# vision-agh/apse_uav

Measured on AMD Instinct MI355X. Metric: 4K UAV frames/sec (whole node), higher is better.
Workload: dtype f32

## Files before the change

### apse_uav_amd/_lib.py

```python
import ctypes as C
import os

import numpy as np

_HERE = os.path.dirname(os.path.abspath(__file__))
_TREE_LIB = os.path.join(_HERE, "libapse_hip.so")
LIB_PATH = os.environ.get("APSE_HIP_LIB") or _TREE_LIB
TOOL_ENTRIES = ("apse_winograd_pack_filter", "apse_winograd_conv2d", "apse_lane_stats")

APSE_OK = 0


class ApseError(RuntimeError):
    pass


class Config(C.Structure):
    _fields_ = [
        ("struct_size", C.c_int), ("device", C.c_int), ("max_batch", C.c_int),
        ("frame_h", C.c_int), ("frame_w", C.c_int), ("image_h", C.c_int), ("image_w", C.c_int),
        ("blocks", C.c_int * 4), ("num_classes", C.c_int),
        ("score_thresh", C.c_float), ("box_nms", C.c_float), ("rpn_nms", C.c_float), ("mask_thresh", C.c_float),
        ("rpn_pre_topk", C.c_int), ("rpn_post_topk", C.c_int), ("dets_per_image", C.c_int),
        ("pixel_mean", C.c_float * 3), ("assoc_roi", C.c_int), ("embed_dim", C.c_int), ("assoc_scale", C.c_float),
        ("compute_dtype", C.c_int), ("storage16", C.c_int),
    ]


class ConfigArch(Config):
    _fields_ = [("arch", C.c_int)]

# ... 44 lines not shown
    "apse_rpn_levels": ([vp, i, i, vp], i),
    "apse_box_head": ([vp, i, vp], i),
    "apse_set_detections": ([vp, vp, vp, vp, vp, i, vp], i),
    "apse_mask_tail": ([vp, i, vp], i),
    "apse_embed": ([vp, i, vp], i),
    "apse_forward": ([vp, i, vp], i),
    "apse_results_describe": ([vp, C.POINTER(ResultsLayout)], i),
    "apse_read_results": ([vp, vp, sz, vp], i),
    "apse_read_results_begin": ([vp, vp, sz, vp], i),
    "apse_read_results_end": ([vp, vp], i),
    "apse_lane_stats": ([vp, C.POINTER(C.c_longlong * 4)], i),
    "apse_copy_mask_window": ([vp, i, i, i, i, i, vp, vp], i),
    "apse_copy_mask_windows": ([vp, i, vp, vp, vp, vp, vp], i),
    "apse_host_copy": ([vp, vp, sz, i], i),
    "apse_feature_shape": ([vp, C.c_char_p, C.POINTER(C.c_int * 3)], i),
    "apse_export_feature": ([vp, C.c_char_p, vp, i, vp], i),
    "apse_debug_tensor": ([vp, C.c_char_p, vp, sz, C.POINTER(sz), vp], i),
    "apse_flops": ([vp, i, C.c_double, C.c_double], C.c_double),
    "apse_profile": ([vp, i], i),
    "apse_profile_read": ([vp, C.POINTER(C.c_double * 42), i], i),
    "apse_conv_packed_elems": ([C.POINTER(ConvDesc)], sz),
    "apse_conv_pack_weight": ([C.POINTER(ConvDesc), vp, i, vp, vp], i),
    "apse_conv2d": ([C.POINTER(ConvDesc), vp, vp, vp, vp, vp, vp, sz, vp], i),
    "apse_winograd_pack_filter": ([vp, i, i, vp], i),
    "apse_winograd_conv2d": ([C.POINTER(ConvDesc), vp, vp, vp, vp, vp], i),
    "apse_maxpool3x3s2": ([vp, vp, i, i, i, i, vp], i),
    "apse_maxpool3x3s2_typed": ([vp, vp, i, i, i, i, i, vp], i),
    "apse_roi_align": ([C.POINTER(vp), C.POINTER(i), C.POINTER(i), vp, i, i, i, vp, vp], i),
    "apse_roi_align_typed": ([C.POINTER(vp), C.POINTER(i), C.POINTER(i), vp, i, i, i, i, vp, vp], i),
    "apse_roi_pool": ([vp, i, i, vp, vp, i, i, f, vp, vp], i),
    "apse_roi_features": ([vp, i, vp, vp, i, i, vp, vp], i),
    "apse_nms_rank": ([vp, vp, vp, i, i, i, i, f, i, vp, vp, vp, vp, vp], i),
    "apse_mask_centroid_dense": ([vp, i, i, C.POINTER(C.c_int * 3), vp], i),
    "apse_mask_closest_dense": ([vp, i, i, f, f, C.POINTER(C.c_int * 2), vp], i),
    "apse_l2_normalize": ([vp, vp, i, i, vp], i),
    "apse_sqdist": ([vp, vp, i, i, i, vp, vp], i),
    "apse_undistort_gamma": ([vp, vp, i, i, i, C.POINTER(C.c_double), C.POINTER(C.c_double), i, vp, i, i, vp], i),
    "apse_lab_tables_host": ([vp, vp, C.c_size_t], C.c_size_t),
    "apse_replay_create": ([i, i, f, i], vp),
    "apse_replay_destroy": ([vp], None),
    "apse_replay_step": ([vp, i, i, vp, vp, vp, C.c_char_p, i, vp], i),
    "apse_replay_packed": ([vp, vp, C.c_longlong, i, i, i, vp, C.c_longlong], C.c_longlong),
    "apse_replay_max_id": ([vp], i),
    "apse_replay_next_id": ([vp], i),
    "apse_render_workspace_bytes": ([i, i, i], sz),
    "apse_render_instances": ([vp, vp, i, i, i, i, vp, i, vp, sz, vp, i, vp, sz, vp], i),
# ... 101 lines not shown
```

### apse_uav_amd/csrc/apse_common.h

```cpp
#pragma once
#include <hip/hip_runtime.h>
#include <stdint.h>

#define APSE_OK 0
#define APSE_E_INVALID (-1)
#define APSE_E_HIP (-2)
#define APSE_E_NOMEM (-3)
#define APSE_E_STATE (-4)
#define APSE_E_MISSING (-5)
#define APSE_MAX_FRAME_W 49152
#define APSE_MAX_FRAME_H 32768
#define APSE_MAX_CLASSES 80
#define APSE_LDS_BYTES 163840

int apse_fail_global(int code, const char* msg);

typedef __attribute__((ext_vector_type(16))) float f32x16;
typedef __attribute__((ext_vector_type(4))) float f32x4;

struct ConvParams {
    const float* x;
    const float* w;
    const uint16_t* w16;
    const float* bias;
// ... 14 lines not shown
    int out_mode;
    int y_ld, y_coff;
    int cdec;
    int splitk;
    int steps_total;
    const void* next_w;
    unsigned next_w_bytes;
    int prec;
    int x_st, res_st, y_st;
    int no_stream;
    const float* wu;
};

int apse_launch_conv(const ConvParams& p, int cfg, hipStream_t s, hipEvent_t ev0 = nullptr, hipEvent_t ev1 = nullptr);
int apse_conv_pick_cfg(int M, int Cout, int steps, int* splitk);
#define APSE_CFG_STREAM 9
#define APSE_CFG_BNECK 10
#define APSE_CFG_GLDS 11
#define APSE_CFG_STEMPOOL 12
#define APSE_CFG_SKINNY 13
#define APSE_NCFG 14
bool apse_conv1x1_stream_ok(const ConvParams& p);
int apse_launch_conv1x1_stream(const ConvParams& p, hipStream_t s, hipEvent_t ev0 = nullptr, hipEvent_t ev1 = nullptr);
bool apse_conv_glds16_ok(const ConvParams& p);
bool apse_conv_glds16_small(const ConvParams& p);
bool apse_conv_skinny_ok(const ConvParams& p);
int apse_launch_conv_skinny(const ConvParams& p, hipStream_t s, hipEvent_t ev0 = nullptr, hipEvent_t ev1 = nullptr);
int apse_launch_conv_glds16(const ConvParams& p, hipStream_t s, hipEvent_t ev0 = nullptr, hipEvent_t ev1 = nullptr);
int apse_conv_effective_cfg(const ConvParams& p, int cfg);
bool apse_conv_winograd_ok(const ConvParams& p, int max_items);
int apse_conv_winograd_blocks(const ConvParams& p);
int apse_launch_conv_winograd(const ConvParams& p, hipStream_t s, hipEvent_t ev0 = nullptr, hipEvent_t ev1 = nullptr);
typedef __bf16 bf16x8 __attribute__((ext_vector_type(8)));

#ifdef __HIPCC__
typedef _Float16 f16x4_t __attribute__((ext_vector_type(4)));
typedef __bf16 bf16x4_t __attribute__((ext_vector_type(4)));
__device__ __forceinline__ f32x4 apse_ld4(const void* base, size_t idx, int st) {
    if (st == 0) return *reinterpret_cast<const f32x4*>(reinterpret_cast<const float*>(base) + idx);
    f32x4 r;
    if (st == 1) {
        const uint2 raw = *reinterpret_cast<const uint2*>(reinterpret_cast<const uint16_t*>(base) + idx);
        r[0] = __uint_as_float(raw.x << 16); r[1] = __uint_as_float(raw.x & 0xffff0000u);
        r[2] = __uint_as_float(raw.y << 16); r[3] = __uint_as_float(raw.y & 0xffff0000u);
    } else {
        const f16x4_t h = *reinterpret_cast<const f16x4_t*>(reinterpret_cast<const uint16_t*>(base) + idx);
// ... 92 lines not shown
```

### apse_uav_amd/csrc/detector.hip

```cpp
#include "detector_ctx.h"

#include <math.h>
#include <string.h>

static std::string g_create_error;

int fail(apse_ctx* c, int code, const std::string& msg) {
    if (c) c->err = msg; else g_create_error = msg;
    return code;
}
int apse_fail_global(int code, const char* msg) { return fail(nullptr, code, msg); }

static int take_event_pair(apse_ctx* c, hipStream_t s) {
    if (!c->prof_on) return -1;
    if (c->ev_used == 0) {
        hipEventRecord(c->ev_pool[c->ev_base], s);
        hipEventRecord(c->ev_pool[c->ev_base + 1], s);
        c->ev_used = 2;
    }
    if (c->ev_used + 2 > APSE_EV_HALF) return -1;
    const int e0 = c->ev_base + c->ev_used;
    c->ev_used += 2;
    return e0;
}
// ... 73 lines not shown
    return APSE_OK;
}

static void count_lane_forward(apse_ctx* c, bool on) {
    if (!on || c->fwd_counted) return;
    ++c->lane_stats[0];
    c->fwd_counted = true;
}

static int run_plan(apse_ctx* c, std::vector<Step>& plan, int batch, hipStream_t s) {
    int* total_dev = reinterpret_cast<int*>(c->res + c->lay.total);
    int* propcnt_dev = reinterpret_cast<int*>(c->res + c->lay.prop_count);
    float* ws = (c->lane && s == c->lane) ? c->ws_lane : c->ws;
    for (size_t si = 0; si < plan.size(); ++si) {
        Step& st = plan[si];
        int rc = APSE_OK;
        if (&plan == &c->backbone && (int)si == c->fpn_step && c->lane && c->tail_live && !event_done(c->tail_ev)) {
            ++c->lane_stats[2];
            HIPCHK(c, hipStreamWaitEvent(s, c->tail_ev, 0));
        }
        if (st.kind == S_CONV) {
            ConvParams p = st.c.p;
            for (size_t sj = si + 1; sj < plan.size() && sj <= si + 2; ++sj)
                if (plan[sj].kind == S_CONV) {
                    const ConvParams& q = plan[sj].c.p;
                    const size_t elems = q.wu ? (size_t)16 * q.Cout * (1 << q.cin_log2) : (size_t)apse_roundup(q.Cout, 128) * q.KH * q.KWCp;
                    p.next_w = q.w16 ? (const void*)q.w16 : (q.wu ? (const void*)q.wu : (const void*)q.w);
                    const size_t bytes = elems * (q.w16 ? 2 : 4);
                    p.next_w_bytes = bytes > (64u << 20) ? (64u << 20) : (unsigned)bytes;
                    break;
                }
            p.B = st.c.fixed_items > 0 ? st.c.fixed_items : batch * st.c.b_mult;
            p.M = p.B * p.OH * p.OW;
            p.ws = ws;
            p.tile_cnt = nullptr;
            p.m_count = nullptr; p.m_per_item = p.OH * p.OW; p.m_hint = 0;
            int cfg = st.c.cfg;
            if (st.c.count_kind == 2) {
                p.m_count = total_dev;
                const int mh = (c->hint_total > 0 ? c->hint_total : 1) * p.m_per_item;
                p.m_hint = mh < p.M ? mh : p.M;
                if (p.prec != 0 && p.splitk == 1 && (cfg == 0 || cfg == 1 || cfg == 3)) {
                    int sk_dyn = 1;
                    const int cfg_dyn = apse_conv_pick_cfg(p.m_hint, p.Cout, p.steps_total, &sk_dyn);
                    if (sk_dyn == 1 && (cfg_dyn == 0 || cfg_dyn == 1 || cfg_dyn == 3)) cfg = cfg_dyn;
                }
            }
            else if (st.c.count_kind == 1 && batch == 1) p.m_count = propcnt_dev;
            const int e0 = take_event_pair(c, s);
            const hipEvent_t ev0 = e0 >= 0 ? c->ev_pool[e0] : nullptr, ev1 = e0 >= 0 ? c->ev_pool[e0 + 1] : nullptr;
            if (st.c.pool_y) {
                rc = apse_k_stem_pool16(p.x, p.w16, p.bias, st.c.pool_y, batch, p.H, p.W, p.prec, s, ev0, ev1);
                cfg = APSE_CFG_STEMPOOL;
            } else if (p.wu) {
                rc = apse_launch_conv_winograd(p, s, ev0, ev1);
            } else {
                rc = apse_launch_conv(p, cfg, s, ev0, ev1);
                cfg = apse_conv_effective_cfg(p, cfg);
            }
            if (e0 >= 0) c->pending.push_back({cfg, st.c.flops_per_item, st.c.count_kind, st.c.b_mult, batch, e0, e0 + 1});
        } else if (st.kind == S_BNECK) {
            const int e0 = take_event_pair(c, s);
            const ConvParams& q1 = st.c.p;
            rc = apse_k_bottleneck64_fused16(st.x, st.p3.res, st.y, q1.w16, q1.bias, st.p2.w16, st.p2.bias, st.p3.w16, st.p3.bias, batch,
                                             st.H, st.W, st.C, st.st, s, e0 >= 0 ? c->ev_pool[e0] : nullptr,
                                             e0 >= 0 ? c->ev_pool[e0 + 1] : nullptr);
            if (e0 >= 0) c->pending.push_back({APSE_CFG_BNECK, st.c.flops_per_item, 0, 1, batch, e0, e0 + 1});
        } else if (st.kind == S_MAXPOOL) {
            rc = apse_k_maxpool3x3s2(st.x, st.y, batch, st.H, st.W, st.C, st.st, s);
        } else {
            rc = apse_k_subsample2(st.x, st.y, batch, st.H, st.W, st.C, st.st, s);
        }
        if (rc != APSE_OK) return fail(c, rc, "launch failed at step " + st.c.name);
    }
    return APSE_OK;
}

int fill_camera(UndistortParams& p, int H, int W, const double* m, const double* dist, int ndist, int do_undistort, int do_gamma) {
    memset(&p, 0, sizeof p);
    if (!m || ndist > 14 || ndist < 0 || (ndist > 0 && !dist)) return APSE_E_INVALID;
    for (int i = 0; i < ndist && i < 12; ++i) p.k[i] = dist[i];
    if (ndist > 12 && (dist[12] != 0.0 || (ndist > 13 && dist[13] != 0.0))) return APSE_E_INVALID;
    const double a = m[0], b = m[1], c = m[2], dd = m[3], e = m[4], f = m[5], g = m[6], h = m[7], k = m[8];
    const double det = a * (e * k - f * h) - b * (dd * k - f * g) + c * (dd * h - e * g);
    if (det == 0.0) return APSE_E_INVALID;
    const double id = 1.0 / det;
    p.ir[0] = (e * k - f * h) * id; p.ir[1] = (c * h - b * k) * id; p.ir[2] = (b * f - c * e) * id;
    p.ir[3] = (f * g - dd * k) * id; p.ir[4] = (a * k - c * g) * id; p.ir[5] = (c * dd - a * f) * id;
    p.ir[6] = (dd * h - e * g) * id; p.ir[7] = (b * g - a * h) * id; p.ir[8] = (a * e - b * dd) * id;
    p.fx = m[0]; p.fy = m[4]; p.u0 = m[2]; p.v0 = m[5];
// ... 674 lines not shown
    else if (nm == "embedding_raw") { src = c->emb_raw; n = (size_t)B * g.dets_per_image * g.embed_dim * 4; }
    else {
        auto it = c->t.find(nm);
        if (it == c->t.end()) return fail(c, APSE_E_MISSING, "no tensor " + nm);
        const Tens& t = it->second;
        int items = B;
        if (nm == "box_pooled" || nm == "box_fc1" || nm == "box_fc2" || nm == "box_pred" || nm == "box_mean" || nm == "box_res5")
            items = B * g.rpn_post_topk;
        else if (nm.rfind("mask_", 0) == 0 || nm.rfind("assoc_", 0) == 0) items = B * g.dets_per_image;
        src = t.p; n = (size_t)items * t.H * t.W * t.C * (t.st ? 2 : 4);
    }
    if (bytes) *bytes = n;
    if (!dst) return APSE_OK;
    if (n > max_bytes) return fail(c, APSE_E_INVALID, "debug buffer too small for " + nm);
    int rc = lane_join(c, (hipStream_t)stream);
    if (rc) return rc;
    HIPCHK(c, hipMemcpyAsync(dst, src, n, hipMemcpyDeviceToDevice, (hipStream_t)stream));
    return lane_follow(c, (hipStream_t)stream);
}

double apse_flops(apse_ctx* c, int batch, double proposals, double detections) {
    if (!c || !c->finalized) return 0.0;
    double f = 0;
    for (auto& s : c->backbone) if (s.kind == S_CONV || s.kind == S_BNECK) f += s.c.flops_per_item * batch;
    for (auto& s : c->rpnhead) f += s.c.flops_per_item * batch;
    for (auto& s : c->c4_res5box) f += s.c.flops_per_item * proposals;
    for (auto& s : c->boxhead) f += s.c.flops_per_item * proposals;
    for (auto& s : c->maskhead) f += s.c.flops_per_item * detections;
    for (auto& s : c->embedfc) f += s.c.flops_per_item * detections;
    return f;
}

int apse_set_camera(apse_ctx* c, const double* m, const double* dist, int ndist, const uint8_t* lut_host, int do_undistort, int do_gamma) {
    if (!c) return APSE_E_INVALID;
    if (lane_drain(c)) return APSE_E_HIP;
    if (!do_undistort && !do_gamma) { c->cam_on = false; return APSE_OK; }
    if (do_gamma && !lut_host) return fail(c, APSE_E_INVALID, "gamma needs a 256-entry LUT");
    UndistortParams p;
    int rc = fill_camera(p, c->cfg.frame_h, c->cfg.frame_w, m, dist, ndist, do_undistort, do_gamma);
    if (rc) return fail(c, rc, "bad camera parameters (3x3 matrix, <= 14 distortion coefficients, tilt terms zero)");
    hipSetDevice(c->cfg.device);
    if (!c->cam_lut) {
        c->cam_lut = dalloc<LabTables>(c, 1);
        if (!c->cam_lut) return fail(c, APSE_E_NOMEM, "camera Lab tables alloc");
    }
    if (lut_host) {
        LabTables host;
// ... 26 lines not shown
```

### apse_uav_amd/csrc/detector_ctx.h

```cpp
#pragma once
#include "apse_kernels.h"
#include "../../include/apse_hip.h"
#include "preproc_pixel.h"

#include <map>
#include <string>
#include <vector>

#define APSE_NARROW_CLASSES 6
#define APSE_EV_HALF 1024

struct HostW { std::vector<float> v; std::vector<int64_t> shape; };
struct Tens { float* p = nullptr; int H = 0, W = 0, C = 0; int st = 0; };

struct ConvStep {
    ConvParams p;
    int b_mult = 1;
    int fixed_items = 0;
    int cfg = 0;
    double flops_per_item = 0;
    int count_kind = 0;
    void* pool_y = nullptr;
    std::string name;
};
enum StepKind { S_CONV, S_MAXPOOL, S_SUBSAMPLE, S_BNECK };
struct Step { StepKind kind; ConvStep c; const float* x; float* y; int H, W, C; int st = 0; ConvParams p2, p3; };

struct apse_ctx {
    apse_config cfg;
    std::string err;
    bool f32_winograd = true;
    std::map<std::string, HostW> hw;
    bool finalized = false;
    int PH = 0, PW = 0;
    std::vector<void*> allocs;
    std::map<std::string, Tens> t;
    std::vector<Step> backbone, rpnhead, boxhead, maskhead, embedfc;
    float* ws = nullptr; size_t ws_floats = 0; int* tile_cnt = nullptr;
    int *hb = nullptr, *hc = nullptr, *vb = nullptr, *vc = nullptr; int hk = 0, vk = 0; uint8_t* rs_tmp = nullptr;
    int rs_pitch = 0;
    int* hcT = nullptr;
    RpnLevels rl_host; RpnLevels* rl_dev = nullptr;
    std::vector<std::vector<TopkJob>> stages; std::vector<TopkJob*> stage_dev; int nslots = 0; uint64_t* lists = nullptr;
    int final_slot_host[5]; int* final_slot_dev = nullptr;
    float *dec_boxes = nullptr, *dec_scores = nullptr; int* dec_valid = nullptr; uint32_t* maxc = nullptr;
    int *keep_idx = nullptr, *keep_cnt = nullptr; void* nms_scratch = nullptr;
    float *props = nullptr, *prop_scores = nullptr; int *prop_entry = nullptr;
    FpnMaps fm;
// ... 68 lines not shown
```

### apse_uav_amd/csrc/ops.hip

```cpp
#include "detector_ctx.h"

#include <string.h>

#include <map>
#include <mutex>
#include <vector>

extern "C" {

size_t apse_conv_packed_elems(const apse_conv_desc* d) {
    const int cin_p = pow2_at_least(d->Cin);
    return (size_t)apse_roundup(d->Cout, 128) * d->KH * apse_roundup(d->KW * cin_p, 32);
}

int apse_conv_pack_weight(const apse_conv_desc* d, const float* w, int cin_real, const float* scale, float* packed) {
    if (!d || !w || !packed) return APSE_E_INVALID;
    const int cin_p = pow2_at_least(d->Cin);
    const int KWCp = apse_roundup(d->KW * cin_p, 32);
    memset(packed, 0, apse_conv_packed_elems(d) * sizeof(float));
    pack_oihw(w, d->Cout, cin_real, d->KH, d->KW, cin_p, scale, packed, KWCp);
    return APSE_OK;
}

int apse_conv2d(const apse_conv_desc* d, const float* x, const float* w, const float* bias, const float* res, float* y, float* ws,
                size_t ws_bytes, void* stream) {
    if (!d || !x || !w || !y) return APSE_E_INVALID;
    const int cin_p = pow2_at_least(d->Cin);
    if (cin_p != d->Cin) return APSE_E_INVALID;
    ConvParams p;
    memset(&p, 0, sizeof p);
    p.x = x; p.w = w; p.bias = bias; p.res = res; p.y = y; p.ws = ws;
    p.B = d->B; p.H = d->H; p.W = d->W; p.cin_log2 = apse_ilog2(cin_p);
    p.KH = d->KH; p.KW = d->KW; p.stride = d->stride; p.pad = d->pad;
    p.KWCp = apse_roundup(d->KW * cin_p, 32);
    p.OH = (d->H + 2 * d->pad - d->KH) / d->stride + 1;
    p.OW = (d->W + 2 * d->pad - d->KW) / d->stride + 1;
    p.Cout = d->Cout; p.relu = d->relu; p.res_mode = d->res_mode;
    p.M = p.B * p.OH * p.OW; p.m_per_item = p.OH * p.OW;
    p.y_ld = d->Cout; p.steps_total = p.KH * (p.KWCp / 32);
    p.prec = (d->prec == 1 || d->prec == 2) ? d->prec : 0;
    p.x_st = d->x_st; p.res_st = d->res_st; p.y_st = d->y_st;
    if (p.x_st < 0 || p.x_st > 2 || p.res_st < 0 || p.res_st > 2 || p.y_st < 0 || p.y_st > 2) return APSE_E_INVALID;
    if (p.prec && p.x_st && p.x_st != p.prec) return APSE_E_INVALID;
    if (p.x_st && cin_p < 8) return APSE_E_INVALID;
    int sk = 1;
    int cfg = apse_conv_pick_cfg(p.M, p.Cout, p.steps_total, &sk);
    if (d->cfg >= 0) { cfg = d->cfg; sk = 1; p.no_stream = (d->cfg != APSE_CFG_STREAM && d->cfg != APSE_CFG_GLDS && d->cfg != APSE_CFG_SKINNY); }
    if (d->splitk > 0) sk = d->splitk;
    if (sk > p.steps_total) sk = p.steps_total;
    p.splitk = sk;
    if (sk > 1 && (size_t)sk * p.M * p.Cout * sizeof(float) > ws_bytes) return APSE_E_INVALID;
    if (sk > 1 && d->fuse_reduce) {
        static int* cnt = nullptr;
        if (!cnt) { if (hipMalloc(reinterpret_cast<void**>(&cnt), 65536 * sizeof(int)) != hipSuccess) return APSE_E_NOMEM; hipMemset(cnt, 0, 65536 * sizeof(int)); }
        p.tile_cnt = cnt;
    }
    if (!p.prec) return apse_launch_conv(p, cfg, (hipStream_t)stream);
    const size_t ne = (size_t)apse_roundup(p.Cout, 128) * p.KH * p.KWCp;
    static uint16_t* d16 = nullptr;
    static size_t d16_cap = 0;
    if (ne > d16_cap) {
        hipDeviceSynchronize();
        if (d16) hipFree(d16);
        d16 = nullptr; d16_cap = 0;
        if (hipMalloc(reinterpret_cast<void**>(&d16), ne * 2) != hipSuccess) return APSE_E_NOMEM;
        d16_cap = ne;
    }
    int rc = apse_k_round16(w, d16, ne, p.prec, (hipStream_t)stream);
    if (rc) return rc;
    p.w16 = d16;
    return apse_launch_conv(p, cfg, (hipStream_t)stream);
}

int apse_winograd_pack_filter(const float* w, int Cout, int Cin, float* packed) {
    if (!w || !packed || Cout < 1 || Cin < 8 || pow2_at_least(Cin) != Cin) return APSE_E_INVALID;
    const std::vector<float> u = winograd_filters(w, Cout, Cin, Cin);
    memcpy(packed, u.data(), u.size() * sizeof(float));
    return APSE_OK;
}

int apse_winograd_conv2d(const apse_conv_desc* d, const float* x, const float* wu, const float* bias, float* y, void* stream) {
    if (!d || !x || !wu || !y || d->B < 1 || d->H < 1 || d->W < 1 || d->Cin < 8 || pow2_at_least(d->Cin) != d->Cin) return APSE_E_INVALID;
    ConvParams p;
    memset(&p, 0, sizeof p);
    p.x = x; p.wu = wu; p.bias = bias; p.y = y;
    p.B = d->B; p.H = d->H; p.W = d->W; p.cin_log2 = apse_ilog2(d->Cin);
    p.KH = d->KH; p.KW = d->KW; p.stride = d->stride; p.pad = d->pad;
    p.OH = d->H; p.OW = d->W; p.Cout = d->Cout; p.relu = d->relu;
    p.M = p.B * p.OH * p.OW; p.m_per_item = p.OH * p.OW;
    p.y_ld = d->Cout; p.splitk = 1;
    p.res_mode = d->res_mode; p.prec = d->prec; p.x_st = d->x_st; p.y_st = d->y_st;
    return apse_launch_conv_winograd(p, (hipStream_t)stream);
}

// ... 181 lines not shown
```

### apse_uav_amd/csrc/plan.hip

```cpp
#include "detector_ctx.h"

#include <math.h>
#include <stdio.h>
#include <string.h>

#define APSE_WINO_MIN_BLOCKS 128
#define APSE_EXPECTED_DETS 8

void pack_oihw(const float* w, int Cout, int Cin, int KH, int KW, int cin_p, const float* scale, float* out, int KWCp) {
    for (int o = 0; o < Cout; ++o) {
        const float sc = scale ? scale[o] : 1.0f;
        for (int r = 0; r < KH; ++r)
            for (int s = 0; s < KW; ++s)
                for (int ci = 0; ci < Cin; ++ci)
                    out[((size_t)o * KH + r) * KWCp + s * cin_p + ci] = w[(((size_t)o * Cin + ci) * KH + r) * KW + s] * sc;
    }
}

static const HostW* getw(apse_ctx* c, const std::string& n) {
    auto it = c->hw.find(n);
    return it == c->hw.end() ? nullptr : &it->second;
}

static Tens make_t(apse_ctx* c, const std::string& name, int items, int H, int W, int C, int st = 0) {
// ... 337 lines not shown
    return add_conv(c, plan, sp3, b2, out);
}

static void fuse_bottleneck16(apse_ctx* c, std::vector<Step>& plan, const std::string& name, const Tens& in, const Tens& out) {
    const size_t n = plan.size();
    const ConvParams &q1 = plan[n - 3].c.p, &q2 = plan[n - 2].c.p, &q3 = plan[n - 1].c.p;
    const int st16 = storage_type(c);
    if (!(st16 && q1.stride == 1 && q1.Cout == 64 && out.C == 256 && (in.C == 64 || in.C == 256) && q1.w16 && q2.w16 && q3.w16 &&
          q1.x_st == st16 && q1.y_st == st16 && q2.y_st == st16 && q3.y_st == st16 && q3.res_st == st16 && q2.KWCp == 192 &&
          q1.KWCp == in.C && q3.KWCp == 64 && (size_t)c->cfg.max_batch * in.H * in.W * in.C * 2 < 0xfffffff0ull &&
          !getenv("APSE_NO_BNECK_FUSE")))
        return;
    Step fs;
    fs.kind = S_BNECK;
    fs.c = plan[n - 3].c;
    fs.c.name = name;
    fs.c.flops_per_item = plan[n - 3].c.flops_per_item + plan[n - 2].c.flops_per_item + plan[n - 1].c.flops_per_item;
    fs.p2 = q2; fs.p3 = q3;
    fs.x = in.p; fs.y = out.p; fs.H = in.H; fs.W = in.W; fs.C = in.C; fs.st = st16;
    plan.resize(n - 3);
    plan.push_back(fs);
}

static Tens add_stem_pool(apse_ctx* c, const Tens& cur) {
    Step st; st.kind = S_MAXPOOL; st.x = cur.p; st.H = cur.H; st.W = cur.W; st.C = cur.C;
    Tens o = make_t(c, "stem", c->cfg.max_batch, (cur.H + 2 - 3) / 2 + 1, (cur.W + 2 - 3) / 2 + 1, cur.C, cur.st);
    st.y = o.p; st.c.name = "stem.pool"; st.st = cur.st;
    c->backbone.push_back(st);
    return o;
}

static int add_mask_predictor(apse_ctx* c, const Tens& in, Tens* logits) {
    const int KD = c->cfg.dets_per_image;
    Tens md;
    ConvSpec dc{"mask_deconv", {"roi_heads.mask_head.deconv"}, 1, 1, 1, 0, 1};
    dc.deconv = 1; dc.items = KD; dc.count_kind = 2;
    int rc = add_conv(c, c->maskhead, dc, in, &md);
    if (rc) return rc;
    ConvSpec ml{"mask_logits", {"roi_heads.mask_head.predictor"}, 1, 1, 1, 0, 0};
    ml.items = KD; ml.count_kind = 2;
    return add_conv(c, c->maskhead, ml, md, logits);
}

static int add_box_predictor(apse_ctx* c, const Tens& in) {
    ConvSpec sp{"box_pred", {"roi_heads.box_predictor.cls_score", "roi_heads.box_predictor.bbox_pred"}, 1, 1, 1, 0, 0};
    sp.items = c->cfg.rpn_post_topk; sp.count_kind = 1;
// ... 27 lines not shown
            sp.out_view = &pooled;
            rc = add_conv(c, c->backbone, sp, x0, &unused);
            if (rc) return rc;
            c->t.erase("stem.conv1");
            c->backbone.back().c.pool_y = pooled.p;
            cur = pooled;
            fused_stem = true;
        } else {
            rc = add_conv(c, c->backbone, sp, x0, &cur);
        }
    } else {
        Tens x0 = make_t(c, "input", B, c->PH, c->PW, 4);
        rc = add_conv(c, c->backbone, ConvSpec{"stem.conv1", {"backbone.bottom_up.stem.conv1"}, 7, 7, 2, 3, 1}, x0, &cur);
    }
    if (rc) return rc;
    if (!fused_stem) cur = add_stem_pool(c, cur);
    for (int si = 0; si < 4; ++si) {
        const std::string stage = "res" + std::to_string(si + 2);
        for (int bi = 0; bi < g.blocks[si]; ++bi) {
            const std::string P = "backbone.bottom_up." + stage + "." + std::to_string(bi);
            const int stride = (bi == 0 && si > 0) ? 2 : 1;
            const bool last = (bi == g.blocks[si] - 1);
            Tens out;
            rc = add_bottleneck(c, c->backbone, P, P, cur, 1, stride, 0, last ? stage : P + ".out", &out);
            if (rc) return rc;
            fuse_bottleneck16(c, c->backbone, P + ".fused", cur, out);
            cur = out;
        }
    }
    c->fpn_step = (int)c->backbone.size();
    Tens inner, pl[5];
    for (int lvl = 5; lvl >= 2; --lvl) {
        char ln[64], on[64], rn[16], in_name[16], pn[8];
        snprintf(ln, sizeof ln, "backbone.fpn_lateral%d", lvl);
        snprintf(on, sizeof on, "backbone.fpn_output%d", lvl);
        snprintf(rn, sizeof rn, "res%d", lvl);
        snprintf(in_name, sizeof in_name, "inner%d", lvl);
        snprintf(pn, sizeof pn, "p%d", lvl);
        Tens ninner;
        ConvSpec lat{ln, {ln}, 1, 1, 1, 0, 0};
        lat.out_name = in_name;
        if (lvl != 5) { lat.res = &inner; lat.res_mode = 2; }
        rc = add_conv(c, c->backbone, lat, c->t[rn], &ninner);
        if (rc) return rc;
        inner = ninner;
        ConvSpec outc{on, {on}, 3, 3, 1, 1, 0};
        outc.out_name = pn;
        rc = add_conv(c, c->backbone, outc, inner, &pl[lvl - 2]);
        if (rc) return rc;
// ... 154 lines not shown
}

int build_plan_c4(apse_ctx* c) {
    const apse_config& g = c->cfg;
    const int B = g.max_batch;
    c->PH = g.image_h;
    c->PW = g.image_w;
    layout_results(c);
    c->res = dalloc<uint8_t>(c, c->lay.bytes);
    if (!c->res) return fail(c, APSE_E_NOMEM, "results alloc");
    int rc;
    Tens cur;
    Tens x0 = make_t(c, "input", B, c->PH, c->PW, 4);
    rc = add_conv(c, c->backbone, ConvSpec{"stem.conv1", {"backbone.stem.conv1"}, 7, 7, 2, 3, 1}, x0, &cur);
    if (rc) return rc;
    cur = add_stem_pool(c, cur);
    for (int si = 0; si < 3; ++si) {
        const std::string stage = "res" + std::to_string(si + 2);
        for (int bi = 0; bi < g.blocks[si]; ++bi) {
            const std::string P = "backbone." + stage + "." + std::to_string(bi);
            const int stride = (bi == 0 && si > 0) ? 2 : 1;
            const bool last = bi == g.blocks[si] - 1;
            Tens out;
            rc = add_bottleneck(c, c->backbone, P, P, cur, 1, stride, 0, last ? stage : P + ".out", &out);
            if (rc) return rc;
            cur = out;
        }
    }
    const Tens res4 = c->t["res4"];
    if (res4.C < 256 || (res4.C & 255)) return fail(c, APSE_E_INVALID, "C4: res4 needs a multiple of 256 channels");
    {
        Tens t, h;
        rc = add_conv(c, c->rpnhead, ConvSpec{"rpn_conv", {"proposal_generator.rpn_head.conv"}, 3, 3, 1, 1, 1}, res4, &t);
        if (rc) return rc;
        ConvSpec sp{"rpn_head", {"proposal_generator.rpn_head.objectness_logits", "proposal_generator.rpn_head.anchor_deltas"},
                    1, 1, 1, 0, 0};
        sp.y_ld = 80;
        rc = add_conv(c, c->rpnhead, sp, t, &h);
        if (rc) return rc;
        if (c->rpnhead.back().c.p.Cout != 75) return fail(c, APSE_E_INVALID, "C4 RPN head: expected 15 objectness + 60 delta channels");
        C4Rpn& R = c->c4r;
        memset(&R, 0, sizeof R);
        R.head = h.p; R.H = h.H; R.W = h.W; R.ld = 80; R.stride = 16;
        R.n = h.H * h.W * 15;
        R.k = R.n < g.rpn_pre_topk ? R.n : g.rpn_pre_topk;
        static const int sizes[5] = {32, 64, 128, 256, 512};
        static const double ratios[3] = {0.5, 1.0, 2.0};
        for (int si = 0; si < 5; ++si)
// ... 28 lines not shown
```

### include/apse_hip.h

```cpp
#ifndef APSE_HIP_H
#define APSE_HIP_H
#include <stddef.h>
#include <stdint.h>
#ifdef __cplusplus
extern "C" {
#endif

#define APSE_OK 0
#define APSE_E_INVALID (-1)
#define APSE_E_HIP (-2)
#define APSE_E_NOMEM (-3)
#define APSE_E_STATE (-4)
#define APSE_E_MISSING (-5)

typedef struct apse_ctx apse_ctx;

#define APSE_MAX_CLASSES 80
#define APSE_C4_MAX_PRE_TOPK 6000
#define APSE_C4_MAX_BATCH 2
#define APSE_MAX_FRAME_W 49152
#define APSE_MAX_FRAME_H 32768
typedef struct apse_config {
    int struct_size;
    int device;
// ... 78 lines not shown
int apse_feature_shape(apse_ctx* ctx, const char* name, int* chw3);
int apse_export_feature(apse_ctx* ctx, const char* name, float* dst_nchw_dev, int batch, void* stream);
int apse_debug_tensor(apse_ctx* ctx, const char* name, void* dst_dev, size_t max_bytes, size_t* bytes, void* stream);
double apse_flops(apse_ctx* ctx, int batch, double proposals, double detections);

int apse_profile(apse_ctx* ctx, int enable);
int apse_profile_read(apse_ctx* ctx, double* out42, int reset);

typedef struct apse_conv_desc {
    int B, H, W, Cin;
    int Cout, KH, KW, stride, pad;
    int relu;
    int res_mode;
    int cfg;
    int splitk;
    int prec;
    int fuse_reduce;
    int x_st, res_st, y_st;
} apse_conv_desc;
size_t apse_conv_packed_elems(const apse_conv_desc* d);
int apse_conv_pack_weight(const apse_conv_desc* d, const float* w_oihw, int cin_real, const float* scale, float* packed);
int apse_conv2d(const apse_conv_desc* d, const float* x_dev, const float* w_packed_dev, const float* bias_dev,
                const float* res_dev, float* y_dev, float* ws_dev, size_t ws_bytes, void* stream);
int apse_winograd_pack_filter(const float* w_oihw, int Cout, int Cin, float* packed);
int apse_winograd_conv2d(const apse_conv_desc* d, const float* x_dev, const float* wu_dev, const float* bias_dev, float* y_dev,
                         void* stream);
int apse_maxpool3x3s2(const float* x_dev, float* y_dev, int B, int H, int W, int C, void* stream);
int apse_maxpool3x3s2_typed(const void* x_dev, void* y_dev, int B, int H, int W, int C, int storage, void* stream);
int apse_roi_align(const float* const* feats_dev, const int* hs, const int* ws, const float* rois_dev, int n, int per_img,
                   int out_size, float* out_dev, void* stream);
int apse_roi_align_typed(const void* const* feats_dev, const int* hs, const int* ws, const float* rois_dev, int n, int per_img,
                         int out_size, int storage, void* out_dev, void* stream);
int apse_roi_pool(const float* feat_dev, int H, int W, const float* rois_dev, const int* roi_img_dev, int n, int out_size,
                  float scale, float* out_dev, void* stream);
int apse_nms_rank(const float* boxes_dev, const float* scores_dev, const int* valid_dev, int n, int cat_div, int cat_mod,
                  int ncat, float thr, int topk, float* out_boxes_dev, float* out_scores_dev, int* out_index_dev,
                  int* out_count_dev, void* stream);
int apse_mask_centroid_dense(const uint8_t* mask_dev, int H, int W, int* out_xy_mass_host3, void* stream);
int apse_mask_closest_dense(const uint8_t* mask_dev, int H, int W, float px, float py, int* out_xy_host2, void* stream);
int apse_l2_normalize(const float* x_dev, float* y_dev, int n, int D, void* stream);
int apse_sqdist(const float* a_dev, const float* b_dev, int O, int N, int D, float* out_dev, void* stream);
int apse_undistort_gamma(const uint8_t* src_dev, uint8_t* dst_dev, int B, int H, int W, const double* mtx3x3_host,
                         const double* dist_host, int ndist, const uint8_t* lut256_host, int do_undistort, int do_gamma,
                         void* stream);
size_t apse_lab_tables_host(const uint8_t* lut256_host, void* out, size_t cap);
int apse_resize_normalize(const uint8_t* frames_dev, uint8_t* tmp_dev, float* out_nhwc4_dev, uint8_t* resized_u8_dev,
// ... 173 lines not shown
```

Baseline: 204.6.

## Fuse bottleneck conv3 with next block's conv1 in one seam kernel

Adds a kernel that computes a bottleneck's final 1x1 expansion conv (bias, residual add, ReLU) and immediately feeds the result, held in LDS, into the next block's 1x1 reduction conv. Both layers run in one launch, so the next block does not re-read the wide activation from memory. The plan builder replaces eligible conv pairs with a new seam step, and the prefetch hint now covers seam steps. By default this applies only to the K=64 stage; the K=128 case needs an environment flag. It adds double-buffered weight staging, higher register pressure and an extra barrier per sub-step.

```diff
diff --git a/apse_uav_amd/_lib.py b/apse_uav_amd/_lib.py
--- a/apse_uav_amd/_lib.py
+++ b/apse_uav_amd/_lib.py
@@ -6,7 +6,7 @@
 _HERE = os.path.dirname(os.path.abspath(__file__))
 _TREE_LIB = os.path.join(_HERE, "libapse_hip.so")
 LIB_PATH = os.environ.get("APSE_HIP_LIB") or _TREE_LIB
-TOOL_ENTRIES = ("apse_winograd_pack_filter", "apse_winograd_conv2d", "apse_lane_stats")
+TOOL_ENTRIES = ("apse_winograd_pack_filter", "apse_winograd_conv2d", "apse_lane_stats", "apse_conv1x1_seam")
 
 APSE_OK = 0
 
@@ -97,6 +97,7 @@
     "apse_conv_packed_elems": ([C.POINTER(ConvDesc)], sz),
     "apse_conv_pack_weight": ([C.POINTER(ConvDesc), vp, i, vp, vp], i),
     "apse_conv2d": ([C.POINTER(ConvDesc), vp, vp, vp, vp, vp, vp, sz, vp], i),
+    "apse_conv1x1_seam": ([C.POINTER(ConvDesc), C.POINTER(ConvDesc), vp, vp, vp, vp, vp, vp, vp, vp, vp], i),
     "apse_winograd_pack_filter": ([vp, i, i, vp], i),
     "apse_winograd_conv2d": ([C.POINTER(ConvDesc), vp, vp, vp, vp, vp], i),
     "apse_maxpool3x3s2": ([vp, vp, i, i, i, i, vp], i),
diff --git a/apse_uav_amd/csrc/apse_common.h b/apse_uav_amd/csrc/apse_common.h
--- a/apse_uav_amd/csrc/apse_common.h
+++ b/apse_uav_amd/csrc/apse_common.h
@@ -60,6 +60,8 @@
 #define APSE_NCFG 14
 bool apse_conv1x1_stream_ok(const ConvParams& p);
 int apse_launch_conv1x1_stream(const ConvParams& p, hipStream_t s, hipEvent_t ev0 = nullptr, hipEvent_t ev1 = nullptr);
+bool apse_conv1x1_seam_ok(const ConvParams& p3, const ConvParams& p1);
+int apse_launch_conv1x1_seam(const ConvParams& p3, const ConvParams& p1, int rows, hipStream_t s, hipEvent_t ev0 = nullptr, hipEvent_t ev1 = nullptr);
 bool apse_conv_glds16_ok(const ConvParams& p);
 bool apse_conv_glds16_small(const ConvParams& p);
 bool apse_conv_skinny_ok(const ConvParams& p);
diff --git a/apse_uav_amd/csrc/conv1x1_seam.hip b/apse_uav_amd/csrc/conv1x1_seam.hip
--- /dev/null
+++ b/apse_uav_amd/csrc/conv1x1_seam.hip
@@ -0,0 +1,265 @@
+#include "apse_common.h"
+
+typedef unsigned sm_u32x4 __attribute__((ext_vector_type(4)));
+
+template <int K3, int N1, int ROWS>
+__global__ __launch_bounds__(ROWS * 2, 2) void conv1x1_seam(const ConvParams p3, const ConvParams p1) {
+    constexpr int NT = ROWS * 2;
+    constexpr int NC = K3 == 64 ? 128 : 64;
+    constexpr int NST3 = K3 / 32;
+    constexpr int NJ3 = NC / 32, NJ1 = N1 / 32;
+    constexpr int SUBS = 128 / N1;
+    constexpr int NST1 = NC / 32 / SUBS;
+    constexpr int SPH = 2 / SUBS;
+    constexpr int SPC = NST3 + NST1;
+    constexpr int RPP = NT / 8;
+    constexpr int NW3 = NC / RPP, NW1 = 128 / RPP;
+    constexpr int CLD = 68;
+    static_assert((K3 == 64 || K3 == 128) && (N1 == 64 || N1 == 128) && (ROWS == 64 || ROWS == 128), "instantiations");
+    static_assert(SPC % 2 == 0 && NST1 * SUBS * 32 == NC && NW3 <= NW1, "stage sequence");
+    extern __shared__ __attribute__((aligned(16))) char smem[];
+    char* Ws = smem;
+    float* Cw = reinterpret_cast<float*>(smem + 2 * 128 * 128);
+
+    const int tid = threadIdx.x, lane = tid & 63, wave = tid >> 6;
+    const int fr = lane & 31, fh = lane >> 5;
+    const int srow = tid >> 3, slot = tid & 7;
+    const int M = p3.M, N3 = p3.Cout;
+    const int m0 = blockIdx.x * ROWS + wave * 32;
+    const int chunks = N3 / NC;
+
+    __amdgpu_buffer_rsrc_t xrsrc = __builtin_amdgcn_make_buffer_rsrc(const_cast<float*>(p3.x), 0, (int)((unsigned)M * (unsigned)K3 * 4u), 0x00020000);
+    f32x4 a[NST3][4];
+    {
+        const int m = m0 + fr;
+#pragma unroll
+        for (int s = 0; s < NST3; ++s)
+#pragma unroll
+            for (int c = 0; c < 4; ++c) {
+                const unsigned off = (m < M) ? (unsigned)m * (unsigned)(K3 * 4) + (unsigned)((s * 32 + (2 * c + fh) * 4) * 4) : 0xfffffff0u;
+                a[s][c] = __builtin_bit_cast(f32x4, __builtin_amdgcn_raw_buffer_load_b128(xrsrc, (int)off, 0, 0));
+            }
+    }
+
+    const float* w3 = p3.w + slot * 4;
+    const float* w1 = p1.w + slot * 4;
+    f32x4 wr[NW1];
+    auto w_fetch = [&](int ch, int t) {
+        if (t >= SPC) { ch += 1; t -= SPC; }
+        if (t < NST3) {
+#pragma unroll
+            for (int i = 0; i < NW3; ++i) {
+                const size_t n = (size_t)ch * NC + srow + RPP * i;
+                wr[i] = *reinterpret_cast<const f32x4*>(w3 + n * K3 + t * 32);
+            }
+        } else {
+            const int u = t - NST3;
+#pragma unroll
+            for (int i = 0; i < NW1; ++i) {
+                const int R = srow + RPP * i, sub = R / N1, n = R - sub * N1;
+                wr[i] = *reinterpret_cast<const f32x4*>(w1 + (size_t)n * N3 + ch * NC + (u * SUBS + sub) * 32);
+            }
+        }
+    };
+    auto w_store = [&](int t) {
+        if (t >= SPC) t -= SPC;
+        const int nw = t < NST3 ? NW3 : NW1;
+#pragma unroll
+        for (int i = 0; i < NW1; ++i)
+            if (i < nw) {
+                const int row = srow + RPP * i;
+                *reinterpret_cast<f32x4*>(Ws + (t & 1) * 128 * 128 + row * 128 + ((slot ^ ((row >> 1) & 7)) << 4)) = wr[i];
+            }
+    };
+    w_fetch(0, 0);
+    w_store(0);
+    w_fetch(0, 1);
+    __syncthreads();
+
+    float* cw = Cw + wave * 32 * CLD;
+    const int erow = lane >> 3, ecol = (lane & 7) * 8;
+    constexpr unsigned DEAD = 0x80000000u;
+    unsigned yrow[4];
+#pragma unroll
+    for (int i = 0; i < 4; ++i) {
+        const int m = m0 + erow + 8 * i;
+        yrow[i] = m < M ? (unsigned)m : DEAD;
+    }
+    const __amdgpu_buffer_rsrc_t yrsrc = __builtin_amdgcn_make_buffer_rsrc(p3.y, 0, (int)((unsigned)M * (unsigned)N3 * 4u), 0x00020000);
+    const __amdgpu_buffer_rsrc_t rrsrc = __builtin_amdgcn_make_buffer_rsrc(const_cast<float*>(p3.res), 0, (int)((unsigned)M * (unsigned)N3 * 4u), 0x00020000);
+    const __amdgpu_buffer_rsrc_t y1rsrc = __builtin_amdgcn_make_buffer_rsrc(p1.y, 0, (int)((unsigned)M * (unsigned)N1 * 4u), 0x00020000);
+    auto row_off = [&](int i, unsigned ld) { return yrow[i] == DEAD ? DEAD : yrow[i] * ld * 4u; };
+
+    constexpr bool RES_AHEAD = K3 == 64 && ROWS == 128;
+    f32x4 rr[4][2];
+    auto load_res = [&](int nb) {
+#pragma unroll
+        for (int i = 0; i < 4; ++i)
+#pragma unroll
+            for (int h2 = 0; h2 < 2; ++h2)
+                rr[i][h2] = __builtin_bit_cast(f32x4, __builtin_amdgcn_raw_buffer_load_b128(rrsrc, (int)(row_off(i, (unsigned)N3) + (unsigned)nb * 4u + h2 * 16u), 0, 0));
+    };
+    if constexpr (RES_AHEAD) load_res(ecol);
+
+    f32x16 acc1[NJ1];
+#pragma unroll
+    for (int j = 0; j < NJ1; ++j)
+#pragma unroll
+        for (int v = 0; v < 16; ++v) acc1[j][v] = 0.f;
+
+    for (int ch = 0; ch < chunks; ++ch) {
+        const bool last = ch + 1 == chunks;
+        auto advance = [&](int t) {
+            if (!(last && t + 1 >= SPC)) w_store(t + 1);
+            if (!(last && t + 2 >= SPC)) w_fetch(ch, t + 2);
+        };
+        f32x16 acc[NJ3];
+#pragma unroll
+        for (int s = 0; s < NST3; ++s) {
+            advance(s);
+            const char* Wb = Ws + (s & 1) * 128 * 128;
+#pragma unroll
+            for (int c = 0; c < 4; ++c) {
+                f32x4 bfr[NJ3];
+                const int ls = 2 * c + fh;
+#pragma unroll
+                for (int j = 0; j < NJ3; ++j) {
+                    const int row = j * 32 + fr;
+                    bfr[j] = *reinterpret_cast<const f32x4*>(Wb + row * 128 + ((ls ^ ((row >> 1) & 7)) << 4));
+                }
+#pragma unroll
+                for (int k = 0; k < 4; ++k)
+#pragma unroll
+                    for (int j = 0; j < NJ3; ++j)
+                        acc[j] = __builtin_amdgcn_mfma_f32_32x32x2f32(a[s][c][k], bfr[j][k], (s == 0 && c == 0 && k == 0) ? f32x16{0.f, 0.f, 0.f, 0.f, 0.f, 0.f, 0.f, 0.f, 0.f, 0.f, 0.f, 0.f, 0.f, 0.f, 0.f, 0.f} : acc[j], 0, 0, 0);
+            }
+            __syncthreads();
+        }
+        const int n0 = ch * NC;
+#pragma unroll
+        for (int hh = 0; hh < NC / 64; ++hh) {
+#pragma unroll
+            for (int q = 0; q < SPH; ++q) {
+                const int t = NST3 + hh * SPH + q;
+                advance(t);
+                if (q == 0) {
+                    const int nb = n0 + hh * 64 + ecol;
+                    if constexpr (!RES_AHEAD) load_res(nb);
+#pragma unroll
+                    for (int jj = 0; jj < 2; ++jj)
+#pragma unroll
+                        for (int v = 0; v < 16; ++v)
+                            cw[((v & 3) + 8 * (v >> 2) + 4 * fh) * CLD + jj * 32 + fr] = acc[2 * hh + jj][v];
+                    __builtin_amdgcn_wave_barrier();
+                    f32x4 b0 = {0.f, 0.f, 0.f, 0.f}, b1 = b0;
+                    if (p3.bias) {
+                        b0 = *reinterpret_cast<const f32x4*>(p3.bias + nb);
+                        b1 = *reinterpret_cast<const f32x4*>(p3.bias + nb + 4);
+                    }
+#pragma unroll
+                    for (int i = 0; i < 4; ++i) {
+                        float* cp = cw + (erow + 8 * i) * CLD + ecol;
+                        f32x4 v0 = *reinterpret_cast<const f32x4*>(cp) + b0;
+                        f32x4 v1 = *reinterpret_cast<const f32x4*>(cp + 4) + b1;
+                        v0 += rr[i][0]; v1 += rr[i][1];
+#pragma unroll
+                        for (int k = 0; k < 4; ++k) { v0[k] = apse_relu(v0[k]); v1[k] = apse_relu(v1[k]); }
+                        const int yoff = (int)(row_off(i, (unsigned)N3) + (unsigned)nb * 4u);
+                        __builtin_amdgcn_raw_buffer_store_b128(__builtin_bit_cast(sm_u32x4, v0), yrsrc, yoff, 0, APSE_NT ? 2 : 0);
+                        __builtin_amdgcn_raw_buffer_store_b128(__builtin_bit_cast(sm_u32x4, v1), yrsrc, yoff + 16, 0, APSE_NT ? 2 : 0);
+                        *reinterpret_cast<f32x4*>(cp) = v0;
+                        *reinterpret_cast<f32x4*>(cp + 4) = v1;
+                    }
+                    __builtin_amdgcn_wave_barrier();
+                    if constexpr (RES_AHEAD)
+                        if (nb - ecol + 64 < N3) load_res(nb + 64);
+                }
+                const char* Wb = Ws + (t & 1) * 128 * 128;
+#pragma unroll
+                for (int sub = 0; sub < SUBS; ++sub) {
+                    const int s2 = (q * SUBS + sub) & 1;
+#pragma unroll
+                    for (int c = 0; c < 4; ++c) {
+                        const int ls = 2 * c + fh;
+                        const f32x4 a1 = *reinterpret_cast<const f32x4*>(cw + fr * CLD + s2 * 32 + ls * 4);
+                        f32x4 bfr[NJ1];
+#pragma unroll
+                        for (int j = 0; j < NJ1; ++j) {
+                            const int row = sub * N1 + j * 32 + fr;
+                            bfr[j] = *reinterpret_cast<const f32x4*>(Wb + row * 128 + ((ls ^ ((row >> 1) & 7)) << 4));
+                        }
+#pragma unroll
+                        for (int k = 0; k < 4; ++k)
+#pragma unroll
+                            for (int j = 0; j < NJ1; ++j)
+                                acc1[j] = __builtin_amdgcn_mfma_f32_32x32x2f32(a1[k], bfr[j][k], acc1[j], 0, 0, 0);
+                    }
+                }
+                if (q == SPH - 1) __builtin_amdgcn_wave_barrier();
+                __syncthreads();
+            }
+        }
+    }
+
+#pragma unroll
+    for (int hh = 0; hh < N1 / 64; ++hh) {
+        const int nb = hh * 64 + ecol;
+#pragma unroll
+        for (int jj = 0; jj < 2; ++jj)
+#pragma unroll
+            for (int v = 0; v < 16; ++v)
+                cw[((v & 3) + 8 * (v >> 2) + 4 * fh) * CLD + jj * 32 + fr] = acc1[2 * hh + jj][v];
+        __builtin_amdgcn_wave_barrier();
+        f32x4 b0 = {0.f, 0.f, 0.f, 0.f}, b1 = b0;
+        if (p1.bias) {
+            b0 = *reinterpret_cast<const f32x4*>(p1.bias + nb);
+            b1 = *reinterpret_cast<const f32x4*>(p1.bias + nb + 4);
+        }
+#pragma unroll
+        for (int i = 0; i < 4; ++i) {
+            const float* cp = cw + (erow + 8 * i) * CLD + ecol;
+            f32x4 v0 = *reinterpret_cast<const f32x4*>(cp) + b0;
+            f32x4 v1 = *reinterpret_cast<const f32x4*>(cp + 4) + b1;
+#pragma unroll
+            for (int k = 0; k < 4; ++k) { v0[k] = apse_relu(v0[k]); v1[k] = apse_relu(v1[k]); }
+            const int yoff = (int)(row_off(i, (unsigned)N1) + (unsigned)nb * 4u);
+            __builtin_amdgcn_raw_buffer_store_b128(__builtin_bit_cast(sm_u32x4, v0), y1rsrc, yoff, 0, APSE_NT ? 2 : 0);
+            __builtin_amdgcn_raw_buffer_store_b128(__builtin_bit_cast(sm_u32x4, v1), y1rsrc, yoff + 16, 0, APSE_NT ? 2 : 0);
+        }
+        __builtin_amdgcn_wave_barrier();
+    }
+}
+
+bool apse_conv1x1_seam_ok(const ConvParams& p3, const ConvParams& p1) {
+    if (p3.prec != 0 || p1.prec != 0 || !apse_conv1x1_stream_ok(p3)) return false;
+    const int K3 = 1 << p3.cin_log2, N1 = p1.Cout;
+    if (!((K3 == 64 && N1 == 64) || (K3 == 128 && N1 == 128))) return false;
+    if (p3.stride != 1 || p3.res_mode != 1 || !p3.res || !p3.relu || (p3.Cout & 127) != 0 || p3.wu) return false;
+    if (p1.KH != 1 || p1.KW != 1 || p1.stride != 1 || p1.pad != 0 || (1 << p1.cin_log2) != p3.Cout || p1.KWCp != p3.Cout) return false;
+    if (p1.x != p3.y || p1.B != p3.B || p1.H != p3.OH || p1.W != p3.OW || p1.OH != p3.OH || p1.OW != p3.OW || p1.M != p3.M) return false;
+    if (!p1.relu || p1.res_mode != 0 || !p1.w || p1.wu || p1.x_st != 0 || p1.y_st != 0) return false;
+    if (p1.out_mode != 0 || p1.y_coff != 0 || p1.y_ld != p1.Cout || p1.splitk != 1 || p1.m_count || p1.tile_cnt) return false;
+    return true;
+}
+
+template <int K3, int N1, int ROWS>
+static int launch_seam(const ConvParams& p3, const ConvParams& p1, hipStream_t s, hipEvent_t ev0, hipEvent_t ev1) {
+    const size_t lds = 2 * 128 * 128 + (ROWS / 32) * 32 * 68 * sizeof(float);
+    static bool attr_done = false;
+    if (!attr_done) {
+        hipFuncSetAttribute(reinterpret_cast<const void*>(&conv1x1_seam<K3, N1, ROWS>), hipFuncAttributeMaxDynamicSharedMemorySize, (int)lds);
+        attr_done = true;
+    }
+    if (ev0) hipEventRecord(ev0, s);
+    hipLaunchKernelGGL((conv1x1_seam<K3, N1, ROWS>), dim3((p3.M + ROWS - 1) / ROWS), dim3(ROWS * 2), lds, s, p3, p1);
+    if (ev1) hipEventRecord(ev1, s);
+    return hipGetLastError() == hipSuccess ? APSE_OK : APSE_E_HIP;
+}
+
+int apse_launch_conv1x1_seam(const ConvParams& p3, const ConvParams& p1, int rows, hipStream_t s, hipEvent_t ev0, hipEvent_t ev1) {
+    const int K3 = 1 << p3.cin_log2;
+    if (!apse_conv1x1_seam_ok(p3, p1) || (rows != 0 && rows != 128 && !(rows == 64 && K3 == 64))) return APSE_E_INVALID;
+    if (K3 == 128) return launch_seam<128, 128, 128>(p3, p1, s, ev0, ev1);
+    if (rows == 0) rows = (p3.M + 127) / 128 < 256 ? 64 : 128;
+    return rows == 128 ? launch_seam<64, 64, 128>(p3, p1, s, ev0, ev1) : launch_seam<64, 64, 64>(p3, p1, s, ev0, ev1);
+}
diff --git a/apse_uav_amd/csrc/detector.hip b/apse_uav_amd/csrc/detector.hip
--- a/apse_uav_amd/csrc/detector.hip
+++ b/apse_uav_amd/csrc/detector.hip
@@ -119,7 +119,7 @@
         if (st.kind == S_CONV) {
             ConvParams p = st.c.p;
             for (size_t sj = si + 1; sj < plan.size() && sj <= si + 2; ++sj)
-                if (plan[sj].kind == S_CONV) {
+                if (plan[sj].kind == S_CONV || plan[sj].kind == S_SEAM) {
                     const ConvParams& q = plan[sj].c.p;
                     const size_t elems = q.wu ? (size_t)16 * q.Cout * (1 << q.cin_log2) : (size_t)apse_roundup(q.Cout, 128) * q.KH * q.KWCp;
                     p.next_w = q.w16 ? (const void*)q.w16 : (q.wu ? (const void*)q.wu : (const void*)q.w);
@@ -163,6 +163,14 @@
                                              st.H, st.W, st.C, st.st, s, e0 >= 0 ? c->ev_pool[e0] : nullptr,
                                              e0 >= 0 ? c->ev_pool[e0 + 1] : nullptr);
             if (e0 >= 0) c->pending.push_back({APSE_CFG_BNECK, st.c.flops_per_item, 0, 1, batch, e0, e0 + 1});
+        } else if (st.kind == S_SEAM) {
+            ConvParams p3 = st.c.p, p1 = st.p2;
+            p3.B = p1.B = batch;
+            p3.M = p3.B * p3.OH * p3.OW; p1.M = p1.B * p1.OH * p1.OW;
+            p3.m_per_item = p3.OH * p3.OW; p1.m_per_item = p1.OH * p1.OW;
+            const int e0 = take_event_pair(c, s);
+            rc = apse_launch_conv1x1_seam(p3, p1, 0, s, e0 >= 0 ? c->ev_pool[e0] : nullptr, e0 >= 0 ? c->ev_pool[e0 + 1] : nullptr);
+            if (e0 >= 0) c->pending.push_back({APSE_CFG_STREAM, st.c.flops_per_item, 0, 1, batch, e0, e0 + 1});
         } else if (st.kind == S_MAXPOOL) {
             rc = apse_k_maxpool3x3s2(st.x, st.y, batch, st.H, st.W, st.C, st.st, s);
         } else {
@@ -883,7 +891,7 @@
 double apse_flops(apse_ctx* c, int batch, double proposals, double detections) {
     if (!c || !c->finalized) return 0.0;
     double f = 0;
-    for (auto& s : c->backbone) if (s.kind == S_CONV || s.kind == S_BNECK) f += s.c.flops_per_item * batch;
+    for (auto& s : c->backbone) if (s.kind == S_CONV || s.kind == S_BNECK || s.kind == S_SEAM) f += s.c.flops_per_item * batch;
     for (auto& s : c->rpnhead) f += s.c.flops_per_item * batch;
     for (auto& s : c->c4_res5box) f += s.c.flops_per_item * proposals;
     for (auto& s : c->boxhead) f += s.c.flops_per_item * proposals;
diff --git a/apse_uav_amd/csrc/detector_ctx.h b/apse_uav_amd/csrc/detector_ctx.h
--- a/apse_uav_amd/csrc/detector_ctx.h
+++ b/apse_uav_amd/csrc/detector_ctx.h
@@ -23,7 +23,7 @@
     void* pool_y = nullptr;
     std::string name;
 };
-enum StepKind { S_CONV, S_MAXPOOL, S_SUBSAMPLE, S_BNECK };
+enum StepKind { S_CONV, S_MAXPOOL, S_SUBSAMPLE, S_BNECK, S_SEAM };
 struct Step { StepKind kind; ConvStep c; const float* x; float* y; int H, W, C; int st = 0; ConvParams p2, p3; };
 
 struct apse_ctx {
diff --git a/apse_uav_amd/csrc/ops.hip b/apse_uav_amd/csrc/ops.hip
--- a/apse_uav_amd/csrc/ops.hip
+++ b/apse_uav_amd/csrc/ops.hip
@@ -22,14 +22,10 @@
     return APSE_OK;
 }
 
-int apse_conv2d(const apse_conv_desc* d, const float* x, const float* w, const float* bias, const float* res, float* y, float* ws,
-                size_t ws_bytes, void* stream) {
-    if (!d || !x || !w || !y) return APSE_E_INVALID;
+static bool conv_params_from_desc(const apse_conv_desc* d, ConvParams& p) {
     const int cin_p = pow2_at_least(d->Cin);
-    if (cin_p != d->Cin) return APSE_E_INVALID;
-    ConvParams p;
+    if (cin_p != d->Cin) return false;
     memset(&p, 0, sizeof p);
-    p.x = x; p.w = w; p.bias = bias; p.res = res; p.y = y; p.ws = ws;
     p.B = d->B; p.H = d->H; p.W = d->W; p.cin_log2 = apse_ilog2(cin_p);
     p.KH = d->KH; p.KW = d->KW; p.stride = d->stride; p.pad = d->pad;
     p.KWCp = apse_roundup(d->KW * cin_p, 32);
@@ -40,9 +36,18 @@
     p.y_ld = d->Cout; p.steps_total = p.KH * (p.KWCp / 32);
     p.prec = (d->prec == 1 || d->prec == 2) ? d->prec : 0;
     p.x_st = d->x_st; p.res_st = d->res_st; p.y_st = d->y_st;
-    if (p.x_st < 0 || p.x_st > 2 || p.res_st < 0 || p.res_st > 2 || p.y_st < 0 || p.y_st > 2) return APSE_E_INVALID;
-    if (p.prec && p.x_st && p.x_st != p.prec) return APSE_E_INVALID;
-    if (p.x_st && cin_p < 8) return APSE_E_INVALID;
+    if (p.x_st < 0 || p.x_st > 2 || p.res_st < 0 || p.res_st > 2 || p.y_st < 0 || p.y_st > 2) return false;
+    if (p.prec && p.x_st && p.x_st != p.prec) return false;
+    if (p.x_st && cin_p < 8) return false;
+    return true;
+}
+
+int apse_conv2d(const apse_conv_desc* d, const float* x, const float* w, const float* bias, const float* res, float* y, float* ws,
+                size_t ws_bytes, void* stream) {
+    if (!d || !x || !w || !y) return APSE_E_INVALID;
+    ConvParams p;
+    if (!conv_params_from_desc(d, p)) return APSE_E_INVALID;
+    p.x = x; p.w = w; p.bias = bias; p.res = res; p.y = y; p.ws = ws;
     int sk = 1;
     int cfg = apse_conv_pick_cfg(p.M, p.Cout, p.steps_total, &sk);
     if (d->cfg >= 0) { cfg = d->cfg; sk = 1; p.no_stream = (d->cfg != APSE_CFG_STREAM && d->cfg != APSE_CFG_GLDS && d->cfg != APSE_CFG_SKINNY); }
@@ -70,6 +75,23 @@
     if (rc) return rc;
     p.w16 = d16;
     return apse_launch_conv(p, cfg, (hipStream_t)stream);
+}
+
+int apse_conv1x1_seam(const apse_conv_desc* d3, const apse_conv_desc* d1, const float* x, const float* w3, const float* b3,
+                      const float* res, float* y3, const float* w1, const float* b1, float* y1, void* stream) {
+    if (!d3 || !d1 || !x || !w3 || !res || !y3 || !w1 || !y1) return apse_fail_global(APSE_E_INVALID, "apse_conv1x1_seam: null argument");
+    ConvParams p3, p1;
+    if (!conv_params_from_desc(d3, p3) || !conv_params_from_desc(d1, p1) || d3->B < 1 || d3->H < 1 || d3->W < 1)
+        return apse_fail_global(APSE_E_INVALID, "apse_conv1x1_seam: bad descriptor");
+    if (d3->splitk > 1 || d1->splitk > 1 || d1->cfg >= 0 || (d3->cfg != -1 && d3->cfg != 64 && d3->cfg != 128))
+        return apse_fail_global(APSE_E_INVALID, "apse_conv1x1_seam: unsplit layers only; d3->cfg is -1, 64 or 128 (rows per block), d1->cfg -1");
+    p3.x = x; p3.w = w3; p3.bias = b3; p3.res = res; p3.y = y3; p3.splitk = 1;
+    p1.x = y3; p1.w = w1; p1.bias = b1; p1.y = y1; p1.splitk = 1;
+    const int rows = d3->cfg < 0 ? 0 : d3->cfg;
+    if (!apse_conv1x1_seam_ok(p3, p1) || (rows == 64 && d3->Cin != 64))
+        return apse_fail_global(APSE_E_INVALID, "apse_conv1x1_seam: not an f32 conv3 (K 64 / 128, same-shape residual, ReLU) + conv1 (1x1, stride 1, "
+                                                "Cin = conv3's Cout, Cout = conv3's K, ReLU) pair this kernel is built for");
+    return apse_launch_conv1x1_seam(p3, p1, rows, (hipStream_t)stream);
 }
 
 int apse_winograd_pack_filter(const float* w, int Cout, int Cin, float* packed) {
diff --git a/apse_uav_amd/csrc/plan.hip b/apse_uav_amd/csrc/plan.hip
--- a/apse_uav_amd/csrc/plan.hip
+++ b/apse_uav_amd/csrc/plan.hip
@@ -383,6 +383,30 @@
     plan.push_back(fs);
 }
 
+static void fuse_seam(apse_ctx* c, std::vector<Step>& plan, size_t first) {
+    if (first == 0 || plan.size() != first + 3 || getenv("APSE_NO_SEAM_FUSE")) return;
+    const Step &s3 = plan[first - 1], &s1 = plan[first];
+    if (s3.kind != S_CONV || s1.kind != S_CONV || s3.c.b_mult != 1 || s1.c.b_mult != 1 || s3.c.count_kind || s1.c.count_kind ||
+        s3.c.fixed_items || s1.c.fixed_items || s3.c.pool_y || s1.c.pool_y)
+        return;
+    ConvParams p3 = s3.c.p, p1 = s1.c.p;
+    p3.B = p1.B = c->cfg.max_batch;
+    p3.M = p3.B * p3.OH * p3.OW; p1.M = p1.B * p1.OH * p1.OW;
+    if (!apse_conv1x1_seam_ok(p3, p1)) return;
+    if (s1.c.cfg != 0 && s1.c.cfg != 1 && s1.c.cfg != 3) return;
+    if ((1 << p3.cin_log2) != 64) {
+        const char* e = getenv("APSE_SEAM_RES3");
+        if (!(e && atoi(e) == 1)) return;
+    }
+    Step fs = s3;
+    fs.kind = S_SEAM;
+    fs.c.name = s3.c.name + "+" + s1.c.name;
+    fs.c.flops_per_item = s3.c.flops_per_item + s1.c.flops_per_item;
+    fs.p2 = s1.c.p;
+    plan[first - 1] = fs;
+    plan.erase(plan.begin() + first);
+}
+
 static Tens add_stem_pool(apse_ctx* c, const Tens& cur) {
     Step st; st.kind = S_MAXPOOL; st.x = cur.p; st.H = cur.H; st.W = cur.W; st.C = cur.C;
     Tens o = make_t(c, "stem", c->cfg.max_batch, (cur.H + 2 - 3) / 2 + 1, (cur.W + 2 - 3) / 2 + 1, cur.C, cur.st);
@@ -456,9 +480,11 @@
             const int stride = (bi == 0 && si > 0) ? 2 : 1;
             const bool last = (bi == g.blocks[si] - 1);
             Tens out;
+            const size_t first = c->backbone.size();
             rc = add_bottleneck(c, c->backbone, P, P, cur, 1, stride, 0, last ? stage : P + ".out", &out);
             if (rc) return rc;
             fuse_bottleneck16(c, c->backbone, P + ".fused", cur, out);
+            fuse_seam(c, c->backbone, first);
             cur = out;
         }
     }
@@ -659,8 +685,10 @@
             const int stride = (bi == 0 && si > 0) ? 2 : 1;
             const bool last = bi == g.blocks[si] - 1;
             Tens out;
+            const size_t first = c->backbone.size();
             rc = add_bottleneck(c, c->backbone, P, P, cur, 1, stride, 0, last ? stage : P + ".out", &out);
             if (rc) return rc;
+            fuse_seam(c, c->backbone, first);
             cur = out;
         }
     }
diff --git a/include/apse_hip.h b/include/apse_hip.h
--- a/include/apse_hip.h
+++ b/include/apse_hip.h
@@ -124,6 +124,9 @@
 int apse_conv_pack_weight(const apse_conv_desc* d, const float* w_oihw, int cin_real, const float* scale, float* packed);
 int apse_conv2d(const apse_conv_desc* d, const float* x_dev, const float* w_packed_dev, const float* bias_dev,
                 const float* res_dev, float* y_dev, float* ws_dev, size_t ws_bytes, void* stream);
+int apse_conv1x1_seam(const apse_conv_desc* d3, const apse_conv_desc* d1, const float* x_dev, const float* w3_packed_dev,
+                      const float* b3_dev, const float* res_dev, float* y3_dev, const float* w1_packed_dev, const float* b1_dev,
+                      float* y1_dev, void* stream);
 int apse_winograd_pack_filter(const float* w_oihw, int Cout, int Cin, float* packed);
 int apse_winograd_conv2d(const apse_conv_desc* d, const float* x_dev, const float* wu_dev, const float* bias_dev, float* y_dev,
                          void* stream);
```

Result: no change. 205.5 (median of 6 runs) (+0.4%).
